# Mamba413/bess

Measured on AMD Instinct MI355X. Metric: candidate subsets solved/sec (n=50k,p=10k,k<=200 LM), higher is better.
Workload: dtype f64; 1 GPU; configs[1]: LM sequential path, Gaussian X n=50000 p=10000, s.list=1..200, GIC, warm start, max_iter=20, is_normal; score_pass=covariance updates (cached Gram columns), collective=none, ranks_with_work=1

## Files before the change

### bess_amd/capi.py

```python
import ctypes
import os
import sys

import numpy as np

_HERE = os.path.dirname(os.path.abspath(__file__))
LIB_PATH = os.environ.get("BESSX_LIB_PATH") or os.path.join(_HERE, "libbessx.so")

_D = ctypes.POINTER(ctypes.c_double)
_I = ctypes.POINTER(ctypes.c_int)
_i = ctypes.c_int
_d = ctypes.c_double
_ll = ctypes.c_longlong
_vp = ctypes.c_void_p

SYMBOLS = [
    "bessx_last_error", "bessx_device_info", "bessx_pywrap_bess", "bessx_bessCpp", "bessx_session_create",
    "bessx_session_destroy", "bessx_session_set_cv", "bessx_session_get_cv_folds", "bessx_session_sequential_path", "bessx_session_gs_path",
    "bessx_session_pgs_path", "bessx_session_get_screening", "bessx_session_get_screening_groups", "bessx_session_get_screening_scores", "bessx_session_score_mode", "bessx_session_counter",
    "bessx_session_trace_enable", "bessx_session_trace_size", "bessx_session_trace_copy_int",
    "bessx_session_trace_copy_double", "bessx_session_get_normalization", "bessx_session_score_pass_stats",
    "bessx_session_enable_kernel_timing", "bessx_session_submodel_steps", "bessx_session_fit", "bessx_session_fit_width", "bessx_session_reset_caches",
    "bessx_session_sequential_path_chain", "bessx_session_cv_eval", "bessx_session_debug_block_stream",
    "bessx_session_set_fill_hook", "bessx_session_set_kpath_chains",
# ... 557 lines not shown
        self._gsize_max = 1
        if gi is not None and gi.size:
            self._gsize_max = int(np.max(np.diff(np.append(gi, self.p))))
        pb = Problem(self.n, self.p, _dp(x), int(x_col_major), _dp(y), _dp(w), data_type, int(is_normal), model_type,
                     algorithm_type, max_iter, int(is_warm_start), _ip(al), al.size, device, _ip(gi),
                     0 if gi is None else gi.size, int(is_screening), int(screening_size), int(score_mode),
                     int(max_sparsity))
        h = _vp()
        if din is not None:
            _check_device_route(lib().bessx_session_create_device(ctypes.byref(h), ctypes.byref(pb), ctypes.byref(din)))
        else:
            _check(lib().bessx_session_create(ctypes.byref(h), ctypes.byref(pb)))
        self._h = h
        self.K = 0
        self.is_warm_start = bool(is_warm_start)
        self.p_kept = lib().bessx_session_get_screening(h, None, 0)

    def score_mode(self):
        return int(lib().bessx_session_score_mode(self._h))

    def counters(self):
        names = {0: "chained_fits", 1: "cg_fallbacks", 2: "passes_over_X", 3: "chained_queued", 7: "cv_side_by_side_rounds",
                 8: "cv_union_fills", 9: "tie_rescues", 10: "cache_restarts", 11: "cv_contexts_dropped",
                 12: "cv_fold_contexts", 13: "shared_wide_fills", 14: "kpath_chunked_paths", 15: "kpath_stitch_refits",
                 16: "kpath_chunk_fills", 17: "kpath_chains_last_path",
                 18: "kpath_stitch_giveups", 19: "group_XTX_ns",
                 22: "kpath_coarse_us",
                 23: "kpath_chunks_us", 24: "kpath_stitch_us", 25: "panel_launches_one_group",
                 26: "panel_ns_one_group", 27: "panel_launches_two_groups", 28: "panel_ns_two_groups",
                 29: "shared_pass_launches", 30: "shared_pass_chain_slots", 31: "shared_pass_partial_batches",
                 32: "own_queue_streams_created_by_the_process", 33: "multi_responses_batched",
                 34: "multi_responses_host", 35: "multi_union_fills", 36: "x_bytes_uploaded_from_host",
                 37: "x_bytes_ingested_on_device", 38: "live_device_bytes_of_the_process",
                 39: "live_pinned_bytes_of_the_process", 40: "allocation_requests_of_the_process"}
        return {n: int(lib().bessx_session_counter(self._h, i)) for i, n in names.items()}

    def screening(self):
        a = np.zeros(self.p_kept, dtype=np.int32)
        lib().bessx_session_get_screening(self._h, _ip(a), a.size)
        return a

    def screening_groups(self):
        n = lib().bessx_session_get_screening_groups(self._h, None, 0)
        a = np.zeros(max(n, 1), dtype=np.int32)
        lib().bessx_session_get_screening_groups(self._h, _ip(a), n)
        return a[:n]

    def screening_scores(self):
        n = lib().bessx_session_get_screening_scores(self._h, None, 0)
        a = np.zeros(max(n, 1))
        lib().bessx_session_get_screening_scores(self._h, _dp(a), n)
        return a[:n]

    def close(self):
        if getattr(self, "_h", None):
            lib().bessx_session_destroy(self._h)
            self._h = None

    def __del__(self):
        try:
            self.close()
        except Exception:
            pass

    def __enter__(self):
        return self

# ... 1872 lines not shown
```

### bess_amd/csrc/bessx_dev.h

```cpp
#ifndef BESSX_DEV_H
#define BESSX_DEV_H

#include <hip/hip_runtime.h>

namespace bessx {

struct FitCtrl {
  int done;
  int l;
  int T0;
  int k_cur;
  int irls_done;
  int irls_steps;
  int info;
  int same_prev;
  double coef0;
  double ll0;
  int d_fresh;
  int irls_last;
  int fast_same;
  int ls_m;
  double ll1;
  int gram_full;
  int cov_nfill;
  int cov_stall;
  int cov_groups;
  int cov_miss;
  int cov_nmiss;
  int serial;
  int sse_valid;
  double sse_dot;
  double sse_nrm;
  unsigned long long snap_seq;
};
static_assert(sizeof(FitCtrl) <= 128, "the published control block is 128 bytes");

// ... 457 lines not shown
hipError_t launch_cov_reduce_compact_sets(const double *part, int p, const int *fcols, const int *slot_of, int *meta,
                                          const CovRowSets &rs, int g0, int ngroups, int nslab, int CS,
                                          const FitCtrl *ctrl, int parked, hipStream_t st);
constexpr int CGB_MAX_K = 4096;
struct CgbState {
  double rr[2];
  double qq;
  int done_step;
  int steps;
};
struct CgbWork {
  double *x, *q, *r[2], *p[2], *ap[2], *part_pq[2], *part_qq;
  CgbState *st;
};
size_t cgb_work_doubles(int kcap);
hipError_t launch_cg_big(const double *G, int p, const int *slot_of, const int *meta, const int *A_new, int k,
                         double ridge, const double *xty, const double *beta_dense, double *work, int kcap, double *sol,
                         FitCtrl *ctrl, int slot, int nsteps, double tol, double yy, hipStream_t st);
struct CovUnion {
  int nf;
  const int *list[8];
  int len[8];
  int on_restart[8];
  int dn;
  const int *const *dlist;
  const int *dlen;
};
hipError_t launch_cov_fill_union(const CovUnion &u, int restart, const int *extras, const double *bd2, int spec_max,
                                 int spec_min, int *slot_of, int *meta, int p, int *fcols, FitCtrl *fill_ctrl,
                                 hipStream_t st, int C = 0);
int cov_streamed_tiles_per_wave();
hipError_t launch_cov_panel(const double *X, const double *aux, long ld, int p, const double *mask, const int *fcols,
                            int g0, int ngroups, int rows_per_slab, int nslab, double *part, const FitCtrl *ctrl,
                            int parked, hipStream_t st);
hipError_t cov_panel_prepare();
hipError_t launch_cov_reduce(const double *part, int p, const int *fcols, const int *slot_of, double *G, int g0,
                             int ngroups, int nslab, const FitCtrl *ctrl, int parked, hipStream_t st,
                             int ex_lo = 0, int ex_hi = 0);
hipError_t launch_rows_permute(const double *X, long ld, int p, const int *perm, long ldp, double *Xp, hipStream_t st);
hipError_t launch_cov_compact(const double *G, int p, const int *slot_of, const int *fcols, int g0, int ngroups,
                              double *GS, int CS, const FitCtrl *ctrl, int parked, hipStream_t st,
                              const double *xtx = nullptr, int *meta = nullptr);
hipError_t launch_cov_d(const double *G, int p, const int *slot_of, const double *xty, const int *A_cur,
                        const double *b_cur, double *d_out, const double *beta_dense, const double *xtx, double n_t,
                        double lambda, const unsigned char *always, double *bd, const unsigned char *inA, double *bmm,
                        const FitCtrl *ctrl, int slot, hipStream_t st);
hipError_t launch_cov_gram(const double *G, int p, const int *slot_of, const int *A_new, int T0, int mt, double *Gt,
                           int *meta, const FitCtrl *ctrl, int slot, hipStream_t st);
hipError_t launch_publish(const unsigned char *dev, unsigned char *host, int ctrl_bytes, size_t off_sse, int n_sse,
                          size_t off_b, size_t off_a, int kcopy, unsigned long long *seq_host, unsigned long long seq,
                          hipStream_t st, const int *count_ptr = nullptr);
hipError_t launch_vec_mul(const double *a, const double *b, long n, double *out, hipStream_t st);
hipError_t launch_part_sum(const double *part, int nrb, int p, double *out, hipStream_t st);
hipError_t launch_fill(double *a, long n, double v, hipStream_t st);
hipError_t launch_gram_cols(const int *A_new, int T0, int mp, int intercept, int rhs_col, int *cols, FitCtrl *ctrl,
                            int slot, const int *A_cur, int allow_skip, hipStream_t st);
hipError_t launch_copy(const double *src, double *dst, long n, hipStream_t st);

}
#endif
```

### bess_amd/csrc/bessx_fit.cpp

```cpp
#include "bessx_host.h"

namespace bessx {

static int score_pass(bessx_session *s, int kind, int rs, int slot, std::vector<std::pair<size_t, bool>> &k1_pairs) {
  if (rs == 0 && shared_pass_applies(s)) {
    if (s->timing) k1_pairs.push_back({(size_t)-1, false});
    if (kind == 2 && s->cox.one_pass)
      return shared_pass_submit(s, nullptr, nullptr, s->part_rs[rs], nullptr, &s->cox, s->ctrl, slot);
    if (kind != 2)
      return shared_pass_submit(s, s->r_rs[rs], kind == 1 ? s->h_rs[rs] : nullptr, s->part_rs[rs],
                                kind == 1 ? s->part2_rs[rs] : nullptr, nullptr, s->ctrl, slot);
  }
  hipEvent_t ea = nullptr, eb = nullptr;
  if (int rc = k1_begin(s, &ea, &eb)) return rc;
  hipError_t e;
  if (kind == 2)
    e = launch_cox_score_pass(s->X, s->ld, s->p, s->U, s->nrb, s->cox, s->part_rs[rs], s->part2_rs[rs], s->ctrl, slot, s->st);
  else
    e = launch_xtv(s->X, s->ld, s->p, s->U, s->r_rs[rs], kind == 1 ? s->h_rs[rs] : nullptr, s->part_rs[rs],
                   kind == 1 ? s->part2_rs[rs] : nullptr, s->ctrl, slot, s->st);
  if (s->timing && e == hipSuccess) {
    e = hipEventRecord(eb, s->st);
    k1_pairs.push_back({s->ev_used - 2, false});
  }
// ... 39 lines not shown
  } else if (e == hipSuccess) {
    int rps_i, nslab_i;
    const int ntask_i = s->gtask_inc_cnt[mt];
    gram_geometry(s, ntask_i * 3, &rps_i, &nslab_i);
    bessx_session::GramCache &gc = s->gcache[rs];
    e = launch_gram_lm_cached(s->X, s->aux, s->ld, s->gcols, s->mask[rs], s->A_new, T0, mt,
                              tasks_full, ntask, rps, nslab, s->gtasks + s->gtask_inc_off[mt],
                              ntask_i, rps_i, nslab_i, s->gpart, s->Gt, s->Rt, s->gsrc, gc.g0, gc.g1, gc.A, gc.meta,
                              s->ctrl, slot, s->st);
    const CholFuse fbz = chol_fallback_only(s);
    if (e == hipSuccess)
      e = launch_chol(s->Gt, T0, mt, lambda, 0, s->xty[rs], s->A_new, s->sol, &s->ctrl->info, s->ctrl, slot, 0, s->st,
                      &fbz);
    if (e == hipSuccess)
      e = launch_sym_fallback(s->Gt, T0, mt, lambda, 0, s->xty[rs], s->A_new, s->sol, &s->ctrl->info, s->ctrl, slot, s->st,
                              &fbz);
  }
  if (e == hipSuccess)
    e = launch_commit(s->ctrl, slot, T0, s->A_new, s->sol, 0, 0, s->A_cur, s->b_cur, s->beta_dense, s->hist,
                      s->hist_beta, s->hist_coef0, s->hist_stride, s->st, s->inA);
  if (e == hipSuccess)
    e = launch_resid_lm(s->X, s->ld, s->n, s->y, s->mask[rs], s->ctrl, slot, s->A_cur, s->b_cur, s->r_rs[rs],
                        s->sse, s->st);
  if (e != hipSuccess) return fail(BESSX_ERR_HIP, std::string("enqueue_lm_slot: ") + hipGetErrorString(e));
  return 0;
}


int enqueue_cov_fill(bessx_session *s, int rs, int ngroups, int parked, const FitCtrl *gate,
                            int gfirst, bool compact, const int *slot_map) {
  bessx_session::CovCache &cv = s->cov[rs];
  const FitCtrl *gc = gate ? gate : s->ctrl;
  const int *smap = slot_map ? slot_map : cv.slot_of;
  for (int g0 = gfirst; g0 < gfirst + ngroups; g0 += COV_SLOT_GROUPS) {
    const int ng = std::min(COV_SLOT_GROUPS, gfirst + ngroups - g0);
    hipEvent_t ea = nullptr, eb = nullptr;
    if (int rc = k1_begin(s, &ea, &eb)) return rc;
    hipError_t e = hipSuccess;
    if (s->cv_shared) {
      const int nsl_all = s->K * s->cvp_nsl;
      e = launch_cov_panel(s->Xp, s->zp, s->ldp, s->p, nullptr, s->cov_fcols, g0, ng, s->cvp_rps, nsl_all, s->cvp_part,
                           gc, parked, s->st);
      if (s->timing && e == hipSuccess) {
        e = hipEventRecord(eb, s->st);
        s->cov_timed.push_back({s->ev_used - 2, g0});
      }
      if (s->K + 1 <= 9 && e == hipSuccess) {
        CovRowSets rsets = {};
        rsets.nr = s->K + 1;
        for (int r = 0; r <= s->K; r++) {
          rsets.G[r] = s->cov[r].G;
          rsets.GS[r] = s->cov[r].GS;
          rsets.xtx[r] = s->xtx[r];
          rsets.ex_lo[r] = r == 0 ? 0 : (r - 1) * s->cvp_nsl;
          rsets.ex_hi[r] = r == 0 ? 0 : r * s->cvp_nsl;
        }
        e = launch_cov_reduce_compact_sets(s->cvp_part, s->p, s->cov_fcols, s->cov[0].slot_of, s->cov[0].meta, rsets, g0, ng,
                                           nsl_all, s->cov_cs, gc, parked, s->st);
      }
      for (int r = 0; r <= s->K && e == hipSuccess && s->K + 1 > 9; r++) {
        bessx_session::CovCache &cr = s->cov[r];
        const int lo = r == 0 ? 0 : (r - 1) * s->cvp_nsl, hi = r == 0 ? 0 : r * s->cvp_nsl;
        e = launch_cov_reduce(s->cvp_part, s->p, s->cov_fcols, cr.slot_of, cr.G, g0, ng, nsl_all, gc, parked, s->st,
                              lo, hi);
        if (e == hipSuccess)
          e = launch_cov_compact(cr.G, s->p, cr.slot_of, s->cov_fcols, g0, ng, cr.GS, s->cov_cs, gc, parked, s->st,
                                 s->xtx[r], cr.meta);
      }
      if (e != hipSuccess) return fail(BESSX_ERR_HIP, std::string("cov panel (shared): ") + hipGetErrorString(e));
      continue;
    }
    e = launch_cov_panel(s->X, s->aux, s->ld, s->p, s->mask[rs], s->cov_fcols, g0, ng, s->cov_rps,
                         s->cov_nslab, s->cov_part, gc, parked, s->st);
    if (s->timing && e == hipSuccess) {
      e = hipEventRecord(eb, s->st);
      s->cov_timed.push_back({s->ev_used - 2, g0});
    }
    if (e == hipSuccess)
      e = launch_cov_reduce(s->cov_part, s->p, s->cov_fcols, smap, cv.G, g0, ng, s->cov_nslab, gc, parked,
                            s->st);
    if (e == hipSuccess && compact)
      e = launch_cov_compact(cv.G, s->p, smap, s->cov_fcols, g0, ng, cv.GS, s->cov_cs, gc, parked, s->st, s->xtx[rs],
                             cv.meta);
    if (e != hipSuccess) return fail(BESSX_ERR_HIP, std::string("cov panel: ") + hipGetErrorString(e));
  }
  return 0;
}

int cov_C_dev(const bessx_session *s) { return s->cov_C - (s->cov_spec - COV_R); }

struct SlotFuse {
  const PubArgs *pub = nullptr;
  bool pub_fused = false;
  bool pub_snapshot = false;
  const PubArgs *attach = nullptr;
  bool attached = false;
  int cont_serial = 0, cont_parent = 0;
  bool cont = false, cont_fused = false;
};

CholFuse cov_fuse_args(bessx_session *s, int rs, int T0, bool force_chol, SlotFuse *sf) {
  bessx_session::CovCache &cv = s->cov[rs];
  CholFuse fz = {cv.G,          cv.slot_of, s->p,         T0,           s->ctrl,        s->A_cur, s->b_cur,
                 s->beta_dense, s->hist,    s->hist_beta, s->hist_coef0, s->hist_stride, s->inA,   s->yy_h[rs],
                 s->part_rs[rs], cv.GS, s->cov_cs,
                 cv.zero, PubArgs{}, s->fb_work, cv.meta + 4};
// ... 1331 lines not shown
```

### bess_amd/csrc/bessx_host.h

```cpp
#ifndef BESSX_HOST_H
#define BESSX_HOST_H
#include <hip/hip_runtime.h>

#include <algorithm>
#include <atomic>
#include <chrono>
#include <cfloat>
#include <cmath>
#include <cstdio>
#include <condition_variable>
#include <cstring>
#include <functional>
#include <mutex>
#include <numeric>
#include <random>
#include <string>
#include <thread>
#include <vector>

#include "../../include/bessx.h"
#include "bessx_dev.h"
#include "bessx_sync.h"

namespace bessx {
// ... 385 lines not shown
    double lambda = 0.0;
    unsigned long long seq = 0;
  } ahead;
  bool chain = true;
  long long chain_queued = 0, chain_hits = 0, chain_dead = 0, chain_mismatch = 0;
  int fit_serial = 0;
  unsigned char *stage_h = nullptr;
  std::vector<double> x_mean_h, x_norm_h;
  std::vector<int> cv_fold;
  std::vector<int> screen_groups, scr_gidx;
  std::vector<double> screen_scores;
  double y_mean_h = 0.0;
  double nullloss = 0.0;
  SparseVec beta;
  double coef0 = 0.0;
  SparseVec beta_init;
  double coef0_init = 0.0;
  int sparsity_level = 0;
  double lambda_level = 0.0;
  int cur_rows = 0;
  int l = 0;
  double sse_train = 0.0, sse_test = 0.0;
  std::vector<SparseVec> cv_init;
  std::vector<int> n_test;
  Trace trace;
  int metric_depth = 0;
  bool timing = false;
  std::vector<hipEvent_t> ev_pool;
  size_t ev_used = 0;
  double k1_seconds = 0.0, k1_bytes = 0.0;
  long long k1_launches = 0;
  double panel_w_seconds[2] = {0.0, 0.0};
  long long panel_w_launches[2] = {0, 0};
  long long n_fits = 0, n_iters = 0;
};

namespace bessx {

static constexpr int COV_R = 32;
static constexpr int COV_SLOT_GROUPS = 2;
static constexpr int COV_CS = 512;

inline Owner &rowset_owner(bessx_session *s, int rs) { return rs == 0 ? s->own : s->cv_own; }

inline int caller_col(const bessx_session *s, int j) { return s->screen_map.empty() ? j : s->screen_map[j]; }

struct SlotFuse;
struct Candidate {
  int T0 = 0;
  double lambda = 0.0;
  SparseVec beta;
  double coef0 = 0.0, loss = 0.0, ic = 0.0;
  int iters = 0;
};
struct PgsArgs;

void ctx_free(bessx_session *c);
void drop_fold_contexts(bessx_session *s);
void session_free(bessx_session *s);
size_t part_elems(const bessx_session *s);
int k1_begin(bessx_session *s, hipEvent_t *a, hipEvent_t *b);
int k1_collect(bessx_session *s, const std::vector<std::pair<size_t, bool>> &pairs);
int cov_collect(bessx_session *s, int nfill);
int alloc_gram_cache(bessx_session *s);
int alloc_cov_cache(bessx_session *s, bool share_map = false);
int reset_path_caches(bessx_session *s);
// ... 57 lines not shown
  std::vector<int> i, A;
  std::vector<double> d, b;
};
bool mc_engine_applies(const bessx_session *s);
int mc_sse_by_residual(bessx_session *c, hipStream_t st, const int *idx, const double *val, int T0, double coef0, double *out);
int mc_contexts(bessx_session *s, int n);
void kchains_contexts(const bessx_session *s, std::vector<bessx_session *> *out);
bessx_session *mc_context(bessx_session *s, int i);
int mc_engine(bessx_session *s, const int *seq, int ns, std::vector<McJob> &jobs, int nrec, double lambda, int width,
              McRecords &rec, std::vector<int> &takeover, long long *fills);
void kchains_quiesce(bessx_session *s);
int kchunks_prepare(bessx_session *s, int ns, bool link, bool link_warm = false);
hipError_t cox_alloc(bessx_session *s);
int chain_ctx_create(bessx_session *ps, bessx_session **out, bool own_queue = true);
int prefill_begin(bessx_session *s, const int *cols, int ncols, int append);
int glm_geometry(bessx_session *s, int T0, int *mt, int *mp, int *ntask, int *ntiles, int *rps, int *nslab);
int enqueue_glm_head(bessx_session *s, int slot, int T0, double lambda, int rs, bool skip_k1,
                            std::vector<std::pair<size_t, bool>> &k1_pairs);
int enqueue_glm_irls_step(bessx_session *s, int slot, int t, int T0, double lambda, int rs);
int enqueue_glm_tail(bessx_session *s, int slot, int T0, int rs);
int cox_reserve(bessx_session *s, int T0);
int enqueue_cox_head(bessx_session *s, int slot, int T0, double lambda, int rs, bool skip_k1,
                            std::vector<std::pair<size_t, bool>> &k1_pairs);
int enqueue_cox_newton(bessx_session *s, int slot, int t, int T0, double lambda, int rs);
int enqueue_cox_tail(bessx_session *s, int slot, int T0, int rs);
PubArgs publish_args(bessx_session *s, int kcopy, int buf, unsigned long long *seq);
PubArgs publish_from_snapshot(const PubArgs &tail);
int publish_flush(bessx_session *s);
int publish_launch(bessx_session *s, const PubArgs &pa);
int publish_enqueue(bessx_session *s, int kcopy, int buf, unsigned long long *seq);
int publish_wait(bessx_session *s, int buf, unsigned long long want);
bool ctx_stream_create(int device, hipStream_t *st, int leave_out = 0, int stride = 1);
long long ctx_streams_created();
void ctx_stream_destroy(hipStream_t st);
bool ctx_streams_own_queue(int device);
int stream_wait_bounded(bessx_session *s, hipStream_t st, const char *what);
int read_results(bessx_session *s, int kcopy = -1);
int algorithm_fit_grouped(bessx_session *s);
int enqueue_chained(bessx_session *s, const bessx_session::Hint &hint, int rs, int parent, int buf, int batch,
                           double parent_lambda, int parent_T0);
int algorithm_fit(bessx_session *s);
void fold_contexts_invalidate(bessx_session *s);
bool side_by_side_applies(const bessx_session *s, int T0);
int fold_fits_side_by_side(bessx_session *s, double *out, const std::vector<int> *only = nullptr,
                                  double *per_fold = nullptr);
double metric_train_loss_value(const bessx_session *s);
double metric_fold_test_loss(const bessx_session *s, int k);
int metric_train_loss(bessx_session *s, double *out);
int metric_test_loss(bessx_session *s, double *out);
int metric_ic(bessx_session *s, int ic_type, int is_cv, double *out);
void denormalize(const bessx_session *s, SparseVec &b, double &coef0, bool gs_variant);
int run_fit(bessx_session *s, int T0, double lambda, const SparseVec &beta_init, double coef0_init);
void store_candidate(bessx_session *s, bessx_path_result *res, const Candidate &c, bool gs_variant);
void store_best(bessx_session *s, bessx_path_result *res, const Candidate &c, bool gs_variant);
bool chain_row_matches(const bessx_session *s, const bessx_path_chain *ch, int row, const Candidate &c);
int sequential_path(bessx_session *s, const int *seq, int ns, const double *lam, int nl, int ic_type,
                           int is_cv, bessx_path_result *res, bessx_path_chain *chain = nullptr);
int gs_path(bessx_session *s, int s_min, int s_max, int ic_type, int is_cv, bessx_path_result *res);
int pgs_path(bessx_session *s, int s_min, int s_max, double lmin, double lmax, int powell_path, int nlambda,
                    int ic_type, int is_cv, bessx_path_result *res);
int settle_device_chain(bessx_session *s);
int run_path(bessx_session *s, bool gs, const int *seq, int ns, const double *lam, int nl, int s_min,
                    int s_max, int ic_type, int is_cv, bessx_path_result *res, const PgsArgs *pgs = nullptr,
                    bessx_path_chain *chain = nullptr);
int need_device();
int upload_padded(Owner &sc, const double *x, int n, int p, int ld_in, int U, double **dX, long *ld_out);
// ... 7 lines not shown
```

### bess_amd/csrc/bessx_k_cov.hip

```cpp
#include "bessx_kdev.hpp"

namespace bessx {

constexpr int COV_NJ = 4;

#ifdef BESSX_PANEL_CLOCK
#define PCLK_BEGIN()                                                  \
  const unsigned long long pclk_t0_ = __builtin_amdgcn_s_memtime();   \
  const unsigned long long pclk_r0_ = __builtin_amdgcn_s_memrealtime()
#define PCLK_END(tag)                                                                                           \
  do {                                                                                                          \
    asm volatile("s_waitcnt vmcnt(0) lgkmcnt(0)" ::: "memory");                                                 \
    if (blockIdx.x == 7 && threadIdx.x == 0) {                                                                  \
      const unsigned long long dt_ = __builtin_amdgcn_s_memtime() - pclk_t0_;                                   \
      const unsigned long long dr_ = __builtin_amdgcn_s_memrealtime() - pclk_r0_;                               \
      printf("PCLK %s cycles %llu ticks100MHz %llu MHz %.0f\n", tag, dt_, dr_, dr_ ? 100.0 * (double)dt_ / (double)dr_ : 0.0); \
    }                                                                                                           \
  } while (0)
#else
#define PCLK_BEGIN()
#define PCLK_END(tag)
#endif

__device__ __forceinline__ bool cov_gate(const FitCtrl *ctrl, int slot) {
  if (ctrl->done) return false;
  if (slot == 0) return ctrl->l == 0;
  return ctrl->l == slot - 1 && !ctrl->same_prev;
}


__global__ void __launch_bounds__(256) k_cov_need(const int *__restrict__ list, int len,
                                                  const double *__restrict__ bd, double *__restrict__ bd2, int p,
                                                  int *__restrict__ slot_of, int *__restrict__ meta, int C,
// ... 139 lines not shown
  for (int i = tot + tid; i < padded; i += 256) fcols[i] = -1;
  for (int i = nm + tid; i < tot; i += 256) slot_of[fcols[i]] = count + i;
  if (tid == 0) {
    meta[0] = count + tot;
    if (restart) {
      meta[3] += 1;
      meta[4] = 0;
    }
    fill_ctrl->cov_stall = 1;
    fill_ctrl->cov_nfill = padded;
    fill_ctrl->cov_groups += padded / COV_R;
    fill_ctrl->k_cur = count + tot;
    fill_ctrl->cov_nmiss = restart;
  }
}

#ifndef DP_PAD
#define DP_PAD 2
#endif
constexpr int DP_RB = 32;
constexpr int DP_LD = DP_RB + DP_PAD;
constexpr int DP_SC = 128;
template <bool MASKED, int NT>
__device__ __forceinline__ void cov_dp_body(const double *__restrict__ X, const double *__restrict__ aux, long ld,
                                            int p, const double *__restrict__ mask, const int *__restrict__ fcols,
                                            int g0, int rows_per_slab, int nslab, int njg,
                                            double *__restrict__ part, double *smem) {
  constexpr int NS = DP_SC / 32;
  constexpr int NL = NS + NT / 2;
  constexpr int COLS = DP_SC + 16 * NT;
  constexpr size_t BUF = (size_t)COLS * DP_LD;
  constexpr int NA = NT / 2, NB = 2;
  const int njg2 = (njg + 1) / 2;
  const int slab = blockIdx.x / njg2, jb = blockIdx.x - slab * njg2;
  const int tid = threadIdx.x, lane = tid & 63, wv = __builtin_amdgcn_readfirstlane(tid >> 6), c = lane & 15, q = lane >> 4;
  const int ta = NT == 4 ? 2 * (wv & 3) : wv, tb = NT == 4 ? 2 * (wv >> 2) : 0;
  const int ru = tid & 15, cbase = tid >> 4;
  const int jc = min(jb * DP_SC + cbase, p - 1);
  const double *sx = X + (size_t)jc * ld + 2 * ru;
  const long sstride = 32 * ld;
  const int ilim = jb * DP_SC + cbase < p ? (p - 1 - (jb * DP_SC + cbase)) / 32 : 0;
  const double *src[NT / 2];
#pragma unroll
  for (int i = 0; i < NT / 2; i++) src[i] = gram_col(X, aux, ld, fcols[g0 * COV_R + i * 32 + cbase]) + 2 * ru;
  const long r_begin = (long)slab * rows_per_slab, r_end = min(r_begin + rows_per_slab, ld);
  const int nchunk = (int)((r_end - r_begin + DP_RB - 1) / DP_RB);
  d2 stA[NL], stB[NL], mA = d2{1.0, 1.0}, mB = d2{1.0, 1.0};
#define DP_LOAD1(st, ms, r, i)                                                                                  \
  do {                                                                                                          \
    if ((i) < NS)                                                                                               \
      st[i] = __builtin_nontemporal_load(reinterpret_cast<const d2 *>(sx + min((i), ilim) * sstride + (r)));    \
    else                                                                                                        \
      st[i] = *reinterpret_cast<const d2 *>(src[(i) >= NS ? (i)-NS : 0] + (r));                                 \
    if (MASKED && (i) == NL - 1) ms = *reinterpret_cast<const d2 *>(mask + (r) + 2 * ru);                       \
  } while (0)
#define DP_STORE1(buf, st, ms, i)                                                                               \
  do {                                                                                                          \
    d2 v__ = st[i];                                                                                             \
    if (MASKED && (i) >= NS) v__ = v__ * ms;                                                                    \
    *reinterpret_cast<d2 *>((buf) + 2 * ru + (size_t)((i)*32 + cbase) * DP_LD) = v__;                           \
  } while (0)
  d4 acc[NA * NB];
#pragma unroll
  for (int t = 0; t < NA * NB; t++) acc[t] = d4{0.0, 0.0, 0.0, 0.0};
  const size_t offa = (size_t)(ta * 16 + c) * DP_LD + 4 * q, offb = (size_t)(DP_SC + tb * 16 + c) * DP_LD + 4 * q;
  struct Ops {
    d2 a0[NA], a1[NA], b0[NB], b1[NB];
  };
  auto read_ops = [&](const double *rows, Ops &o) {
#pragma unroll
    for (int a = 0; a < NA; a++) {
      o.a0[a] = *reinterpret_cast<const d2 *>(rows + offa + (size_t)a * 16 * DP_LD);
      o.a1[a] = *reinterpret_cast<const d2 *>(rows + offa + (size_t)a * 16 * DP_LD + 2);
    }
#pragma unroll
    for (int t = 0; t < NB; t++) {
      o.b0[t] = *reinterpret_cast<const d2 *>(rows + offb + (size_t)t * 16 * DP_LD);
      o.b1[t] = *reinterpret_cast<const d2 *>(rows + offb + (size_t)t * 16 * DP_LD + 2);
    }
  };
#define DP_MFMA(o, j)                                                                                           \
  do {                                                                                                          \
    _Pragma("unroll") for (int a__ = 0; a__ < NA; a__++) {                                                    \
      const double av__ = (j) == 0 ? (o).a0[a__].x : ((j) == 1 ? (o).a0[a__].y : ((j) == 2 ? (o).a1[a__].x : (o).a1[a__].y)); \
      _Pragma("unroll") for (int t__ = 0; t__ < NB; t__++) {                                                  \
        const double bv__ = (j) == 0 ? (o).b0[t__].x : ((j) == 1 ? (o).b0[t__].y : ((j) == 2 ? (o).b1[t__].x : (o).b1[t__].y)); \
        acc[a__ * NB + t__] = __builtin_amdgcn_mfma_f64_16x16x4f64(av__, bv__, acc[a__ * NB + t__], 0, 0, 0);   \
      }                                                                                                         \
    }                                                                                                           \
  } while (0)
  static_assert(DP_RB == 32, "two row steps per chunk");
#define DP_STEP(o, s, nxt, st, ms, rload)                                                                       \
  do {                                                                                                          \
    int n__ = (s) * NL;                                                                                         \
    _Pragma("unroll") for (int j__ = 0; j__ < 4; j__++) {                                                     \
      DP_MFMA(o, j__);                                                                                          \
                                         \
      const int due__ = (2 * NL * ((s) * 4 + j__ + 1)) / (4 * (DP_RB / 16));                                    \
      _Pragma("unroll") for (int k__ = 0; k__ < 2 * NL; k__++) {                                              \
        if (k__ >= n__ && k__ < due__) {                                                                        \
          if (k__ < NL)                                                                                         \
            DP_STORE1(nxt, st, ms, k__);                                                                        \
          else                                                                                                  \
            DP_LOAD1(st, ms, rload, k__ - NL);                                                                  \
        }                                                                                                       \
      }                                                                                                         \
      n__ = due__;                                                                                              \
      __builtin_amdgcn_sched_barrier(0);                                                                        \
    }                                                                                                           \
  } while (0)
#define DP_CHUNK(cur, nxt, st, ms, rload)                                                                       \
  do {                                                                                                          \
    read_ops((cur) + 16, ob);                                                                                   \
    __builtin_amdgcn_sched_barrier(0);                                                                          \
    DP_STEP(oa, 0, nxt, st, ms, rload);                                                                         \
    __syncthreads();                                                                                            \
    read_ops(nxt, oa);                                                                                          \
    __builtin_amdgcn_sched_barrier(0);                                                                          \
    DP_STEP(ob, 1, nxt, st, ms, rload);                                                                         \
  } while (0)
  double *buf0 = smem, *buf1 = smem + BUF;
  const long r_last = r_begin + (long)(nchunk - 1) * DP_RB;
#pragma unroll
  for (int i = 0; i < NL; i++) DP_LOAD1(stA, mA, r_begin, i);
#pragma unroll
  for (int i = 0; i < NL; i++) DP_STORE1(buf0, stA, mA, i);
  {
    const long r1 = min(r_begin + DP_RB, r_last), r2 = min(r_begin + 2 * DP_RB, r_last);
#pragma unroll
    for (int i = 0; i < NL; i++) DP_LOAD1(stB, mB, r1, i);
#pragma unroll
    for (int i = 0; i < NL; i++) DP_LOAD1(stA, mA, r2, i);
  }
  __syncthreads();
  Ops oa, ob;
  read_ops(buf0, oa);
  for (int k = 0; k < nchunk; k += 2) {
    {
      const long rl = min(r_begin + (long)(k + 3) * DP_RB, r_last);
      DP_CHUNK(buf0, buf1, stB, mB, rl);
    }
    if (k + 1 >= nchunk) break;
    {
      const long rl = min(r_begin + (long)(k + 4) * DP_RB, r_last);
      DP_CHUNK(buf1, buf0, stA, mA, rl);
    }
  }
#undef DP_STEP
#undef DP_CHUNK
#undef DP_MFMA
#undef DP_LOAD1
#undef DP_STORE1
  const size_t tiles_per_slab = (size_t)njg * COV_NJ * 2;
#pragma unroll
  for (int a = 0; a < NA; a++) {
    const int jg = 2 * jb + ((ta + a) >> 2);
    if (jg < njg) {
#pragma unroll
      for (int t = 0; t < NB; t++) {
        double *out = part + (((size_t)((tb + t) >> 1) * nslab + slab) * tiles_per_slab + (size_t)(jg * COV_NJ + ((ta + a) & 3)) * 2 + ((tb + t) & 1)) * 256;
        *reinterpret_cast<d4 *>(out + lane * 4) = acc[a * NB + t];
      }
    }
  }
}

template <bool MASKED>
__global__ void __launch_bounds__(512, 1) k_cov_panel_dp(const double *__restrict__ X, const double *__restrict__ aux,
                                                         long ld, int p, const double *__restrict__ mask,
                                                         const int *__restrict__ fcols, int g0, int ngroups,
                                                         int rows_per_slab, int nslab, int njg,
                                                         double *__restrict__ part, const FitCtrl *__restrict__ ctrl,
                                                         int big) {
  KT(5);
  if (big ? !ctrl->cov_stall : (ctrl->done || ctrl->l != 0)) return;
  const int nfill = ctrl->cov_nfill;
  if (g0 * COV_R >= nfill) return;
  extern __shared__ double smem[];
  PCLK_BEGIN();
  if (ngroups >= 2 && (g0 + 1) * COV_R < nfill)
    cov_dp_body<MASKED, 4>(X, aux, ld, p, mask, fcols, g0, rows_per_slab, nslab, njg, part, smem);
  else
    cov_dp_body<MASKED, 2>(X, aux, ld, p, mask, fcols, g0, rows_per_slab, nslab, njg, part, smem);
  PCLK_END("dp");
}

__device__ __forceinline__ void cov_reduce_body(const double *__restrict__ part, int g0, int ngroups, int nslab,
                                                int njg, int p, const int *__restrict__ fcols,
                                                const int *__restrict__ slot_of, double *__restrict__ G,
                                                const FitCtrl *__restrict__ ctrl, int big,
                                                int ex_lo, int ex_hi) {
  if (big ? !ctrl->cov_stall : (ctrl->done || ctrl->l != 0)) return;
  const int gl = blockIdx.y;
  if (gl >= ngroups || (g0 + gl) * COV_R >= ctrl->cov_nfill) return;
  const size_t tiles_per_slab = (size_t)njg * COV_NJ * 2;
  const int tile = blockIdx.x, e = threadIdx.x;
  double s = 0.0;
// ... 216 lines not shown
hipError_t launch_cov_publish_slots(const int *fcols, const int *slot_w, int *slot_of, const FitCtrl *ctrl, hipStream_t st) {
  hipLaunchKernelGGL(k_cov_publish_slots, dim3(1), dim3(256), 0, st, fcols, slot_w, slot_of, ctrl);
  LAUNCH_CHECK();
  return hipSuccess;
}

hipError_t launch_cov_fill_list(int *fcols, const int *extras, const double *bd2, int *slot_of, int *meta,
                                FitCtrl *ctrl, int parked, hipStream_t st, int spec_max, int spec, int spec_min) {
  if (spec_min <= 0) spec_min = spec_max / 2;
  hipLaunchKernelGGL(k_cov_fill_list, dim3(1), dim3(256), 0, st, fcols, extras, bd2, slot_of, meta, ctrl, parked,
                     spec_max, spec, spec_min);
  LAUNCH_CHECK();
  return hipSuccess;
}

hipError_t launch_cov_resume(FitCtrl *ctrl, hipStream_t st) {
  hipLaunchKernelGGL(k_cov_resume, dim3(1), dim3(1), 0, st, ctrl);
  LAUNCH_CHECK();
  return hipSuccess;
}

hipError_t launch_cov_fill_union(const CovUnion &u, int restart, const int *extras, const double *bd2, int spec_max,
                                 int spec_min, int *slot_of, int *meta, int p, int *fcols, FitCtrl *fill_ctrl,
                                 hipStream_t st, int C) {
  if (u.nf < 1 || u.nf > 8 || u.dn < 0 || (u.dn > 0 && (!u.dlist || !u.dlen)) || spec_max > 64 || spec_min < 0 || spec_min > spec_max) return hipErrorInvalidValue;
  hipLaunchKernelGGL(k_cov_fill_union, dim3(1), dim3(256), 0, st, u, restart, extras, bd2, spec_max, spec_min, slot_of, meta, p,
                     fcols, fill_ctrl, C);
  LAUNCH_CHECK();
  return hipSuccess;
}

int cov_streamed_tiles_per_wave() { return COV_NJ; }

hipError_t launch_cov_panel(const double *X, const double *aux, long ld, int p, const double *mask, const int *fcols,
                            int g0, int ngroups, int rows_per_slab, int nslab, double *part, const FitCtrl *ctrl,
                            int parked, hipStream_t st) {
  if (ngroups < 1 || ngroups > 2) return hipErrorInvalidValue;
  const int pt = (p + 15) / 16, njg = (pt + COV_NJ - 1) / COV_NJ;
  const size_t ldsd = (size_t)2 * (DP_SC + 64) * DP_LD * sizeof(double);
  const long nbd = (long)nslab * ((njg + 1) / 2);
  if (mask)
    hipLaunchKernelGGL(k_cov_panel_dp<true>, dim3((unsigned)nbd), dim3(512), ldsd, st, X, aux, ld, p, mask, fcols, g0,
                       ngroups, rows_per_slab, nslab, njg, part, ctrl, parked);
  else
    hipLaunchKernelGGL(k_cov_panel_dp<false>, dim3((unsigned)nbd), dim3(512), ldsd, st, X, aux, ld, p, mask, fcols, g0,
                       ngroups, rows_per_slab, nslab, njg, part, ctrl, parked);
  LAUNCH_CHECK();
  return hipSuccess;
}

hipError_t cov_panel_prepare() {
  const int ldsd = (int)((size_t)2 * (DP_SC + 64) * DP_LD * sizeof(double));
  hipError_t e = hipFuncSetAttribute(reinterpret_cast<const void *>(&k_cov_panel_dp<true>),
                                     hipFuncAttributeMaxDynamicSharedMemorySize, ldsd);
  if (e != hipSuccess) return e;
  return hipFuncSetAttribute(reinterpret_cast<const void *>(&k_cov_panel_dp<false>),
                             hipFuncAttributeMaxDynamicSharedMemorySize, ldsd);
}

hipError_t launch_cov_reduce(const double *part, int p, const int *fcols, const int *slot_of, double *G, int g0,
                             int ngroups, int nslab, const FitCtrl *ctrl, int parked, hipStream_t st, int ex_lo,
                             int ex_hi) {
  const int pt = (p + 15) / 16, njg = (pt + COV_NJ - 1) / COV_NJ;
  hipLaunchKernelGGL(k_cov_reduce, dim3(njg * COV_NJ * 2, ngroups), dim3(256), 0, st, part, g0, ngroups, nslab, njg, p,
                     fcols, slot_of, G, ctrl, 0, parked, ex_lo, ex_hi);
  LAUNCH_CHECK();
  return hipSuccess;
}

hipError_t launch_cov_reduce_compact_sets(const double *part, int p, const int *fcols, const int *slot_of, int *meta,
                                          const CovRowSets &rs, int g0, int ngroups, int nslab, int CS,
                                          const FitCtrl *ctrl, int parked, hipStream_t st) {
  if (rs.nr < 1 || rs.nr > 9) return hipErrorInvalidValue;
  const int pt = (p + 15) / 16, njg = (pt + COV_NJ - 1) / COV_NJ;
  hipLaunchKernelGGL(k_cov_reduce_sets, dim3(njg * COV_NJ * 2, ngroups, rs.nr), dim3(256), 0, st, part, g0, ngroups,
                     nslab, njg, p, fcols, slot_of, rs, ctrl, parked);
  LAUNCH_CHECK();
  hipLaunchKernelGGL(k_cov_compact_sets, dim3((p + 255) / 256, ngroups, rs.nr), dim3(256), 0, st, rs, p, slot_of, fcols,
// ... 59 lines not shown
```

### bess_amd/csrc/bessx_session.cpp

```cpp
#include "bessx_host.h"

namespace bessx {

thread_local std::string g_err;
thread_local int g_marginal_fit_variant = 0;



void ctx_free(bessx_session *c) {
  if (!c) return;
  if (c->st) (void)hipStreamSynchronize(c->st);
  c->own.release();
  if (c->st) ctx_stream_destroy(c->st);
  delete c;
}

void drop_fold_contexts(bessx_session *s) {
  if (s->fold_pool) {
    s->fold_pool->stop();
    if (!s->fold_pool->broken) delete s->fold_pool;
    s->fold_pool = nullptr;
  }
  for (bessx_session *c : s->fold_ctx) ctx_free(c);
  s->fold_ctx.clear();
// ... 157 lines not shown
    for (auto &o : g_own_streams)
      if (!o.in_use && o.device == device && o.leave_out == leave_out && o.stride == stride) {
        o.in_use = true;
        *st = o.st;
        return true;
      }
    if (g_own_streams.size() >= std::max(cap, OWN_QUEUE_CAP)) {
      for (size_t i = 0; i < g_own_streams.size(); i++)
        if (!g_own_streams[i].in_use) {
          (void)hipStreamDestroy(g_own_streams[i].st);
          g_own_streams.erase(g_own_streams.begin() + (long)i);
          break;
        }
      if (g_own_streams.size() >= std::max(cap, OWN_QUEUE_CAP)) return false;
    }
  }
  hipDeviceProp_t prop;
  if (hipGetDeviceProperties(&prop, device) != hipSuccess || prop.multiProcessorCount <= 0) return false;
  std::vector<uint32_t> mask((size_t)(prop.multiProcessorCount + 31) / 32, 0xffffffffu);
  if (prop.multiProcessorCount % 32) mask.back() = (1u << (prop.multiProcessorCount % 32)) - 1u;
  for (int i = 0; i < leave_out; i++) {
    const int bit = (int)(((long)i * std::max(1, stride)) % prop.multiProcessorCount);
    mask[(size_t)bit / 32] &= ~(1u << (bit % 32));
  }
  if (hipExtStreamCreateWithCUMask(st, (uint32_t)mask.size(), mask.data()) != hipSuccess) {
    (void)hipGetLastError();
    *st = nullptr;
    return false;
  }
  std::lock_guard<std::mutex> lk(g_own_mu);
  g_own_streams.push_back({*st, device, leave_out, stride, true});
  g_own_created++;
  return true;
}

bool ctx_streams_own_queue(int device) {
  static std::mutex mu;
  static std::vector<int> known;
  std::lock_guard<std::mutex> lk(mu);
  if (device < 0) return false;
  if ((int)known.size() <= device) known.resize((size_t)device + 1, -1);
  if (known[(size_t)device] < 0) {
    hipStream_t st = nullptr;
    const bool ok = ctx_stream_create(device, &st);
    if (ok) ctx_stream_destroy(st);
    known[(size_t)device] = ok ? 1 : 0;
  }
  return known[(size_t)device] == 1;
}

int stream_wait_bounded(bessx_session *s, hipStream_t st, const char *what) {
  const auto t0 = std::chrono::steady_clock::now();
  for (unsigned spins = 0;; spins++) {
    const hipError_t q = hipStreamQuery(st);
    if (q == hipSuccess) return 0;
    if (q != hipErrorNotReady) return fail(BESSX_ERR_HIP, std::string(what) + ": " + hipGetErrorString(q));
    if (std::chrono::duration<double>(std::chrono::steady_clock::now() - t0).count() > s->wait_deadline_s)
      return fail(BESSX_ERR_HIP, std::string(what) + ": the stream did not drain within " +
                                     std::to_string(s->wait_deadline_s) + " s (BESSX_WAIT_TIMEOUT_S) -- the session can "
                                     "only be destroyed now");
    if (spins > 2000) std::this_thread::sleep_for(std::chrono::microseconds(50));
  }
}

int reset_path_caches(bessx_session *s) {
  kchains_quiesce(s);
// ... 814 lines not shown
      if (C >= 2 * COV_R + s->cov_spec) {
        s->cov_mode = true;
        s->cov_C = (int)C;
        const int pt = (p + 15) / 16, njg = (pt + cov_streamed_tiles_per_wave() - 1) / cov_streamed_tiles_per_wave();
        long ns = 1, rps = ld;
        long panel_blocks = 0;
        {
          const long conc = 256;
          double best = 1e300;
          const long ns_max = std::max<long>(1, std::min<long>(64, ld / 256));
          for (long t = 1; t <= ns_max; t++) {
            const long r = ((ld + t - 1) / t + 63) / 64 * 64, used = (ld + r - 1) / r;
            const long blocks = (long)((njg + 1) / 2) * used;
            const double cost = (double)((blocks + conc - 1) / conc) * (double)r * (blocks < conc ? 2.0 : 1.0);
            if (cost < best) {
              best = cost;
              ns = used;
              rps = r;
              panel_blocks = blocks;
            }
          }
        }
        s->cov_panel_blocks = (int)std::min<long>(panel_blocks, 1 << 30);
        s->cov_rps = (int)rps;
        s->cov_nslab = (int)ns;
        HIPT(s->own.alloc(&s->cov_part, (size_t)COV_SLOT_GROUPS * ns * njg * cov_streamed_tiles_per_wave() * 2 * 256));
        HIPT(s->own.alloc(&s->bd2, (size_t)p));
        HIPT(s->own.zeros(&s->inA, (size_t)p));
        HIPT(s->own.alloc(&s->cov_bmm, (size_t)3 * ((p + 31) / 32)));
        HIPT(s->own.alloc(&s->cov_fcols, (size_t)s->capA + 4 * COV_R));
        HIPT(s->own.alloc(&s->cov_extras, (size_t)2 * COV_R));
        TRY(alloc_cov_cache(s));
        HIPT(cov_panel_prepare());
        if (const char *ev = test_hook("cov_solver")) s->cov_cg = std::string(ev) != "chol";
        if (const char *ev = test_hook("fuse")) s->fuse = std::string(ev) != "0";
        if (const char *ev = test_hook("fuse_sel")) s->fuse_sel = std::string(ev) != "0";
        if (const char *ev = test_hook("defer_publish")) s->defer_pub = std::string(ev) != "0";
        if (!s->fuse) s->defer_pub = false;
        if (const char *ev = test_hook("cg_layout")) s->cg_by_rows = std::string(ev) != "tiles";
        if (const char *ev = test_hook("cov_cs")) s->cov_cs = std::min(COV_CS, std::max(1, std::atoi(ev)));
      } else if (mode == 2) {
        return bail(fail(BESSX_ERR_ARG, "covariance score mode: p too large for the Gram column cache"));
      }
    }
  }
  HIPT(s->own.alloc(&s->idcols, (size_t)capA + 16));
  if (s->model_type == 4) HIPT(cox_alloc(s));
  if (s->model_type == 1) {
    TRY(prepare_rowset(s, 0));
    if (const char *ev = test_hook("path_group_xtx")) s->path_group_xtx = std::string(ev) != "0";
  }
  HIPT(hipStreamSynchronize(s->st));
#undef TRY
#undef HIPT
  *out = s;
  return BESSX_OK;
}

static int fetch_device_vector(const char *what, const void *data, int dtype, long long stride, int n, int device,
                               hipStream_t caller, std::vector<double> &host) {
  int dev = -1;
  if (int rc = check_device_matrix(what, data, dtype, stride, 0, n, 1, &dev)) return rc;
  if (dev != device) return fail(BESSX_ERR_ARG, std::string(what) + ": memory of another device than the session's");
  const long long ld = ((long long)n + 127) / 128 * 128;
  Owner sc;
  double *d = nullptr;
// ... 524 lines not shown
    case 4: return 0;
    case 5:
    case 6: return 0;
    case 7: return s->cv_rounds;
    case 8: return s->cv_union_fills;
    case 9: return s->cov_tie_rescues;
    case 11: return s->cv_ctx_dropped;
    case 12: return (long long)s->fold_ctx.size();
    case 13: return s->shared_wide_fills;
    case 14: return s->kch_paths;
    case 15: return s->kch_refits;
    case 16: return s->kch_chunk_fills;
    case 17: return s->kch_last_chains;
    case 18: return s->kch_giveups;
    case 19: {
      if (s->xtx_ev_pending && s->xtx_ev[0] && s->xtx_ev[1]) {
        float ms = 0.f;
        bessx_session *w = const_cast<bessx_session *>(s);
        if (hipEventSynchronize(s->xtx_ev[1]) == hipSuccess && hipEventElapsedTime(&ms, s->xtx_ev[0], s->xtx_ev[1]) == hipSuccess)
          w->group_xtx_ns = (long long)(1e6 * (double)ms);
        w->xtx_ev_pending = false;
      }
      return s->group_xtx_ns;
    }
    case 20:
    case 21: return 0;
    case 22: return (long long)(1e6 * s->kch_t[0]);
    case 23: return (long long)(1e6 * s->kch_t[1]);
    case 24: return (long long)(1e6 * s->kch_t[2]);
    case 25: return s->panel_w_launches[0];
    case 26: return (long long)(1e9 * s->panel_w_seconds[0]);
    case 27: return s->panel_w_launches[1];
    case 28: return (long long)(1e9 * s->panel_w_seconds[1]);
    case 29: return s->sp_launches;
    case 30: return s->sp_chain_slots;
    case 31: return s->sp_partial;
    case 32: return ctx_streams_created();
    case 33: return s->multi_batched;
    case 34: return s->multi_host;
    case 35: return s->multi_fills;
    case 36: return s->x_host_bytes;
    case 37: return s->x_dev_bytes;
    case 38: return Ledger::device_bytes.load();
    case 39: return Ledger::pinned_bytes.load();
    case 40: return Ledger::requests.load();
    case 10: {
      if (s->cov.empty()) return 0;
      int m[8] = {0, 0, 0, 0, 0, 0, 0, 0};
      if (hipSetDevice(s->device) != hipSuccess || hipStreamSynchronize(s->st) != hipSuccess ||
          hipMemcpy(m, s->cov[0].meta, sizeof(m), hipMemcpyDeviceToHost) != hipSuccess)
        return -1;
      return m[3];
    }
    default: return -1;
  }
}

int bessx_session_get_screening(const bessx_session *s, int *columns, int cap) {
  if (!s) return 0;
  for (int j = 0; j < s->p && j < cap && columns; j++) columns[j] = caller_col(s, j);
  return s->p;
}

int bessx_session_get_screening_groups(const bessx_session *s, int *groups, int cap) {
  if (!s) return 0;
  const int cnt = (int)s->screen_groups.size();
// ... 31 lines not shown
```

Baseline: 19140 candidates/s.

## Make covariance panel kernel persistent with grid-stride work items

The covariance panel kernel now launches at most one workgroup per compute unit and walks (slab, column-block) items in a grid-stride loop. It carries the double-buffered prefetch across item boundaries, so the next item's loads overlap the current item's tail, and it stores each item's accumulators when that item finishes. This targets launch tail effects and pipeline refill cost from many short workgroups. The cost is more complex control flow, possible extra register pressure, and load imbalance when items do not divide evenly across workgroups.

```diff
diff --git a/bess_amd/capi.py b/bess_amd/capi.py
--- a/bess_amd/capi.py
+++ b/bess_amd/capi.py
@@ -613,7 +613,8 @@
                  32: "own_queue_streams_created_by_the_process", 33: "multi_responses_batched",
                  34: "multi_responses_host", 35: "multi_union_fills", 36: "x_bytes_uploaded_from_host",
                  37: "x_bytes_ingested_on_device", 38: "live_device_bytes_of_the_process",
-                 39: "live_pinned_bytes_of_the_process", 40: "allocation_requests_of_the_process"}
+                 39: "live_pinned_bytes_of_the_process", 40: "allocation_requests_of_the_process",
+                 41: "panel_workgroups_last_launch", 42: "panel_items_last_launch"}
         return {n: int(lib().bessx_session_counter(self._h, i)) for i, n in names.items()}
 
     def screening(self):
diff --git a/bess_amd/csrc/bessx_dev.h b/bess_amd/csrc/bessx_dev.h
--- a/bess_amd/csrc/bessx_dev.h
+++ b/bess_amd/csrc/bessx_dev.h
@@ -2,6 +2,8 @@
 #define BESSX_DEV_H
 
 #include <hip/hip_runtime.h>
+
+#include "bessx_panel_items.h"
 
 namespace bessx {
 
@@ -525,7 +527,8 @@
 int cov_streamed_tiles_per_wave();
 hipError_t launch_cov_panel(const double *X, const double *aux, long ld, int p, const double *mask, const int *fcols,
                             int g0, int ngroups, int rows_per_slab, int nslab, double *part, const FitCtrl *ctrl,
-                            int parked, hipStream_t st);
+                            int parked, hipStream_t st, int grid);
+int cov_panel_items(int p, int nslab);
 hipError_t cov_panel_prepare();
 hipError_t launch_cov_reduce(const double *part, int p, const int *fcols, const int *slot_of, double *G, int g0,
                              int ngroups, int nslab, const FitCtrl *ctrl, int parked, hipStream_t st,
diff --git a/bess_amd/csrc/bessx_fit.cpp b/bess_amd/csrc/bessx_fit.cpp
--- a/bess_amd/csrc/bessx_fit.cpp
+++ b/bess_amd/csrc/bessx_fit.cpp
@@ -95,6 +95,12 @@
   bessx_session::CovCache &cv = s->cov[rs];
   const FitCtrl *gc = gate ? gate : s->ctrl;
   const int *smap = slot_map ? slot_map : cv.slot_of;
+  const int units = ctx_stream_units(s->device, s->st);
+  auto grid_of = [&](int nslab) {
+    s->panel_last_items = cov_panel_items(s->p, nslab);
+    s->panel_last_grid = panel_grid(s->panel_last_items, units, s->panel_grid_cap);
+    return s->panel_last_grid;
+  };
   for (int g0 = gfirst; g0 < gfirst + ngroups; g0 += COV_SLOT_GROUPS) {
     const int ng = std::min(COV_SLOT_GROUPS, gfirst + ngroups - g0);
     hipEvent_t ea = nullptr, eb = nullptr;
@@ -103,7 +109,7 @@
     if (s->cv_shared) {
       const int nsl_all = s->K * s->cvp_nsl;
       e = launch_cov_panel(s->Xp, s->zp, s->ldp, s->p, nullptr, s->cov_fcols, g0, ng, s->cvp_rps, nsl_all, s->cvp_part,
-                           gc, parked, s->st);
+                           gc, parked, s->st, grid_of(nsl_all));
       if (s->timing && e == hipSuccess) {
         e = hipEventRecord(eb, s->st);
         s->cov_timed.push_back({s->ev_used - 2, g0});
@@ -134,7 +140,7 @@
       continue;
     }
     e = launch_cov_panel(s->X, s->aux, s->ld, s->p, s->mask[rs], s->cov_fcols, g0, ng, s->cov_rps,
-                         s->cov_nslab, s->cov_part, gc, parked, s->st);
+                         s->cov_nslab, s->cov_part, gc, parked, s->st, grid_of(s->cov_nslab));
     if (s->timing && e == hipSuccess) {
       e = hipEventRecord(eb, s->st);
       s->cov_timed.push_back({s->ev_used - 2, g0});
diff --git a/bess_amd/csrc/bessx_host.h b/bess_amd/csrc/bessx_host.h
--- a/bess_amd/csrc/bessx_host.h
+++ b/bess_amd/csrc/bessx_host.h
@@ -441,6 +441,8 @@
   long long k1_launches = 0;
   double panel_w_seconds[2] = {0.0, 0.0};
   long long panel_w_launches[2] = {0, 0};
+  int panel_last_grid = 0, panel_last_items = 0;
+  int panel_grid_cap = 0;
   long long n_fits = 0, n_iters = 0;
 };
 
@@ -564,6 +566,7 @@
 int publish_wait(bessx_session *s, int buf, unsigned long long want);
 bool ctx_stream_create(int device, hipStream_t *st, int leave_out = 0, int stride = 1);
 long long ctx_streams_created();
+int ctx_stream_units(int device, hipStream_t st);
 void ctx_stream_destroy(hipStream_t st);
 bool ctx_streams_own_queue(int device);
 int stream_wait_bounded(bessx_session *s, hipStream_t st, const char *what);
diff --git a/bess_amd/csrc/bessx_k_cov.hip b/bess_amd/csrc/bessx_k_cov.hip
--- a/bess_amd/csrc/bessx_k_cov.hip
+++ b/bess_amd/csrc/bessx_k_cov.hip
@@ -1,4 +1,5 @@
 #include "bessx_kdev.hpp"
+#include "bessx_panel_items.h"
 
 namespace bessx {
 
@@ -204,24 +205,52 @@
   constexpr size_t BUF = (size_t)COLS * DP_LD;
   constexpr int NA = NT / 2, NB = 2;
   const int njg2 = (njg + 1) / 2;
-  const int slab = blockIdx.x / njg2, jb = blockIdx.x - slab * njg2;
+  const int G = (int)gridDim.x, items = panel_item_count(nslab, njg2);
   const int tid = threadIdx.x, lane = tid & 63, wv = __builtin_amdgcn_readfirstlane(tid >> 6), c = lane & 15, q = lane >> 4;
   const int ta = NT == 4 ? 2 * (wv & 3) : wv, tb = NT == 4 ? 2 * (wv >> 2) : 0;
   const int ru = tid & 15, cbase = tid >> 4;
-  const int jc = min(jb * DP_SC + cbase, p - 1);
-  const double *sx = X + (size_t)jc * ld + 2 * ru;
   const long sstride = 32 * ld;
-  const int ilim = jb * DP_SC + cbase < p ? (p - 1 - (jb * DP_SC + cbase)) / 32 : 0;
+  auto chunks_of = [&](int slab) {
+    const long rb = (long)slab * rows_per_slab;
+    return (int)((min(rb + rows_per_slab, ld) - rb + DP_RB - 1) / DP_RB);
+  };
+  const double *cp[NS];
+  auto columns_of = [&](int jb) {
+    const int j0 = jb * DP_SC + cbase;
+    const double *sx = X + (size_t)min(j0, p - 1) * ld + 2 * ru;
+    const int ilim = j0 < p ? (p - 1 - j0) / 32 : 0;
+#pragma unroll
+    for (int i = 0; i < NS; i++) cp[i] = sx + min(i, ilim) * sstride;
+  };
+  int item_l = panel_item_of((int)blockIdx.x, 0, G), item_c = item_l;
+  if (item_c >= items) return;
+  PanelItem it_c = panel_item_split(item_c, njg2);
+  int rem_c = chunks_of(it_c.slab), rem_l = rem_c;
+  long r_l = (long)it_c.slab * rows_per_slab;
+  columns_of(it_c.jb);
+  auto advance_load = [&]() {
+    r_l += DP_RB;
+    if (--rem_l == 0) {
+      if (item_l + G < items) {
+        item_l += G;
+        const PanelItem it = panel_item_split(item_l, njg2);
+        r_l = (long)it.slab * rows_per_slab;
+        rem_l = chunks_of(it.slab);
+        columns_of(it.jb);
+      } else {
+        r_l -= DP_RB;
+        rem_l = 1;
+      }
+    }
+  };
   const double *src[NT / 2];
 #pragma unroll
   for (int i = 0; i < NT / 2; i++) src[i] = gram_col(X, aux, ld, fcols[g0 * COV_R + i * 32 + cbase]) + 2 * ru;
-  const long r_begin = (long)slab * rows_per_slab, r_end = min(r_begin + rows_per_slab, ld);
-  const int nchunk = (int)((r_end - r_begin + DP_RB - 1) / DP_RB);
   d2 stA[NL], stB[NL], mA = d2{1.0, 1.0}, mB = d2{1.0, 1.0};
 #define DP_LOAD1(st, ms, r, i)                                                                                  \
   do {                                                                                                          \
     if ((i) < NS)                                                                                               \
-      st[i] = __builtin_nontemporal_load(reinterpret_cast<const d2 *>(sx + min((i), ilim) * sstride + (r)));    \
+      st[i] = __builtin_nontemporal_load(reinterpret_cast<const d2 *>(cp[(i) < NS ? (i) : 0] + (r)));           \
     else                                                                                                        \
       st[i] = *reinterpret_cast<const d2 *>(src[(i) >= NS ? (i)-NS : 0] + (r));                                 \
     if (MASKED && (i) == NL - 1) ms = *reinterpret_cast<const d2 *>(mask + (r) + 2 * ru);                       \
@@ -281,6 +310,7 @@
       __builtin_amdgcn_sched_barrier(0);                                                                        \
     }                                                                                                           \
   } while (0)
+#define DP_FENCE() asm volatile("" ::: "memory")
 #define DP_CHUNK(cur, nxt, st, ms, rload)                                                                       \
   do {                                                                                                          \
     read_ops((cur) + 16, ob);                                                                                   \
@@ -290,51 +320,64 @@
     read_ops(nxt, oa);                                                                                          \
     __builtin_amdgcn_sched_barrier(0);                                                                          \
     DP_STEP(ob, 1, nxt, st, ms, rload);                                                                         \
+    DP_FENCE();                                                                                                 \
   } while (0)
   double *buf0 = smem, *buf1 = smem + BUF;
-  const long r_last = r_begin + (long)(nchunk - 1) * DP_RB;
-#pragma unroll
-  for (int i = 0; i < NL; i++) DP_LOAD1(stA, mA, r_begin, i);
+  const size_t tiles_per_slab = (size_t)njg * COV_NJ * 2;
+  auto store_item = [&](const PanelItem &it) {
+#pragma unroll
+    for (int a = 0; a < NA; a++) {
+      const int jg = 2 * it.jb + ((ta + a) >> 2);
+      if (jg < njg) {
+#pragma unroll
+        for (int t = 0; t < NB; t++) {
+          double *out = part + (((size_t)((tb + t) >> 1) * nslab + it.slab) * tiles_per_slab + (size_t)(jg * COV_NJ + ((ta + a) & 3)) * 2 + ((tb + t) & 1)) * 256;
+          *reinterpret_cast<d4 *>(out + lane * 4) = acc[a * NB + t];
+        }
+      }
+    }
+  };
+#pragma unroll
+  for (int i = 0; i < NL; i++) DP_LOAD1(stA, mA, r_l, i);
+  advance_load();
 #pragma unroll
   for (int i = 0; i < NL; i++) DP_STORE1(buf0, stA, mA, i);
-  {
-    const long r1 = min(r_begin + DP_RB, r_last), r2 = min(r_begin + 2 * DP_RB, r_last);
-#pragma unroll
-    for (int i = 0; i < NL; i++) DP_LOAD1(stB, mB, r1, i);
-#pragma unroll
-    for (int i = 0; i < NL; i++) DP_LOAD1(stA, mA, r2, i);
-  }
+#pragma unroll
+  for (int i = 0; i < NL; i++) DP_LOAD1(stB, mB, r_l, i);
+  DP_FENCE();
+  advance_load();
+#pragma unroll
+  for (int i = 0; i < NL; i++) DP_LOAD1(stA, mA, r_l, i);
+  DP_FENCE();
+  advance_load();
   __syncthreads();
   Ops oa, ob;
   read_ops(buf0, oa);
-  for (int k = 0; k < nchunk; k += 2) {
-    {
-      const long rl = min(r_begin + (long)(k + 3) * DP_RB, r_last);
-      DP_CHUNK(buf0, buf1, stB, mB, rl);
-    }
-    if (k + 1 >= nchunk) break;
-    {
-      const long rl = min(r_begin + (long)(k + 4) * DP_RB, r_last);
-      DP_CHUNK(buf1, buf0, stA, mA, rl);
-    }
-  }
+#define DP_ITEM_END()                                                                                           \
+  if (--rem_c == 0) {                                                                                           \
+    store_item(it_c);                                                                                           \
+    item_c += G;                                                                                                \
+    more = item_c < items;                                                                                      \
+    _Pragma("unroll") for (int t__ = 0; t__ < NA * NB; t__++) acc[t__] = d4{0.0, 0.0, 0.0, 0.0};              \
+    it_c = panel_item_split(more ? item_c : 0, njg2);                                                           \
+    rem_c = more ? chunks_of(it_c.slab) : 0x7fffffff;                                                           \
+  }
+  bool more = true;
+  do {
+    DP_CHUNK(buf0, buf1, stB, mB, r_l);
+    advance_load();
+    DP_ITEM_END();
+    DP_CHUNK(buf1, buf0, stA, mA, r_l);
+    advance_load();
+    DP_ITEM_END();
+  } while (more);
+#undef DP_ITEM_END
 #undef DP_STEP
 #undef DP_CHUNK
+#undef DP_FENCE
 #undef DP_MFMA
 #undef DP_LOAD1
 #undef DP_STORE1
-  const size_t tiles_per_slab = (size_t)njg * COV_NJ * 2;
-#pragma unroll
-  for (int a = 0; a < NA; a++) {
-    const int jg = 2 * jb + ((ta + a) >> 2);
-    if (jg < njg) {
-#pragma unroll
-      for (int t = 0; t < NB; t++) {
-        double *out = part + (((size_t)((tb + t) >> 1) * nslab + slab) * tiles_per_slab + (size_t)(jg * COV_NJ + ((ta + a) & 3)) * 2 + ((tb + t) & 1)) * 256;
-        *reinterpret_cast<d4 *>(out + lane * 4) = acc[a * NB + t];
-      }
-    }
-  }
 }
 
 template <bool MASKED>
@@ -617,18 +660,24 @@
 
 int cov_streamed_tiles_per_wave() { return COV_NJ; }
 
+int cov_panel_items(int p, int nslab) {
+  const int pt = (p + 15) / 16, njg = (pt + COV_NJ - 1) / COV_NJ;
+  return panel_item_count(nslab, (njg + 1) / 2);
+}
+
 hipError_t launch_cov_panel(const double *X, const double *aux, long ld, int p, const double *mask, const int *fcols,
                             int g0, int ngroups, int rows_per_slab, int nslab, double *part, const FitCtrl *ctrl,
-                            int parked, hipStream_t st) {
+                            int parked, hipStream_t st, int grid) {
   if (ngroups < 1 || ngroups > 2) return hipErrorInvalidValue;
   const int pt = (p + 15) / 16, njg = (pt + COV_NJ - 1) / COV_NJ;
+  const int items = cov_panel_items(p, nslab);
+  if (grid < 1 || grid > items || rows_per_slab < 1 || (long)(nslab - 1) * rows_per_slab >= ld) return hipErrorInvalidValue;
   const size_t ldsd = (size_t)2 * (DP_SC + 64) * DP_LD * sizeof(double);
-  const long nbd = (long)nslab * ((njg + 1) / 2);
   if (mask)
-    hipLaunchKernelGGL(k_cov_panel_dp<true>, dim3((unsigned)nbd), dim3(512), ldsd, st, X, aux, ld, p, mask, fcols, g0,
+    hipLaunchKernelGGL(k_cov_panel_dp<true>, dim3((unsigned)grid), dim3(512), ldsd, st, X, aux, ld, p, mask, fcols, g0,
                        ngroups, rows_per_slab, nslab, njg, part, ctrl, parked);
   else
-    hipLaunchKernelGGL(k_cov_panel_dp<false>, dim3((unsigned)nbd), dim3(512), ldsd, st, X, aux, ld, p, mask, fcols, g0,
+    hipLaunchKernelGGL(k_cov_panel_dp<false>, dim3((unsigned)grid), dim3(512), ldsd, st, X, aux, ld, p, mask, fcols, g0,
                        ngroups, rows_per_slab, nslab, njg, part, ctrl, parked);
   LAUNCH_CHECK();
   return hipSuccess;
diff --git a/bess_amd/csrc/bessx_panel_items.h b/bess_amd/csrc/bessx_panel_items.h
--- /dev/null
+++ b/bess_amd/csrc/bessx_panel_items.h
@@ -0,0 +1,35 @@
+#pragma once
+
+#if defined(__HIPCC__) || defined(__CUDACC__)
+#define BESSX_HD __host__ __device__
+#else
+#define BESSX_HD
+#endif
+
+namespace bessx {
+
+struct PanelItem {
+  int slab, jb;
+};
+
+BESSX_HD inline int panel_item_count(int nslab, int blocks_per_slab) { return nslab * blocks_per_slab; }
+
+BESSX_HD inline int panel_grid(int items, int units, int cap) {
+  int g = items;
+  if (units > 0 && g > units) g = units;
+  if (cap > 0 && g > cap) g = cap;
+  return g < 1 ? 1 : g;
+}
+
+BESSX_HD inline int panel_item_of(int w, int t, int G) { return w + t * G; }
+
+BESSX_HD inline int panel_items_of_workgroup(int items, int G, int w) { return w < items ? (items - 1 - w) / G + 1 : 0; }
+
+BESSX_HD inline PanelItem panel_item_split(int item, int blocks_per_slab) {
+  PanelItem it;
+  it.slab = item / blocks_per_slab;
+  it.jb = item - it.slab * blocks_per_slab;
+  return it;
+}
+
+}
diff --git a/bess_amd/csrc/bessx_session.cpp b/bess_amd/csrc/bessx_session.cpp
--- a/bess_amd/csrc/bessx_session.cpp
+++ b/bess_amd/csrc/bessx_session.cpp
@@ -213,6 +213,30 @@
   g_own_streams.push_back({*st, device, leave_out, stride, true});
   g_own_created++;
   return true;
+}
+
+int ctx_stream_units(int device, hipStream_t st) {
+  static std::mutex mu;
+  static std::vector<int> cus;
+  int n = 0;
+  {
+    std::lock_guard<std::mutex> lk(mu);
+    if (device < 0) return 0;
+    if ((int)cus.size() <= device) cus.resize((size_t)device + 1, 0);
+    if (cus[(size_t)device] == 0) {
+      hipDeviceProp_t prop;
+      if (hipGetDeviceProperties(&prop, device) != hipSuccess || prop.multiProcessorCount <= 0) {
+        (void)hipGetLastError();
+        return 0;
+      }
+      cus[(size_t)device] = prop.multiProcessorCount;
+    }
+    n = cus[(size_t)device];
+  }
+  std::lock_guard<std::mutex> lk(g_own_mu);
+  for (auto &o : g_own_streams)
+    if (o.st == st && o.in_use) return std::max(1, n - std::min(o.leave_out, n));
+  return n;
 }
 
 bool ctx_streams_own_queue(int device) {
@@ -1093,6 +1117,7 @@
         HIPT(s->own.alloc(&s->cov_extras, (size_t)2 * COV_R));
         TRY(alloc_cov_cache(s));
         HIPT(cov_panel_prepare());
+        if (const char *ev = test_hook("panel_grid")) s->panel_grid_cap = std::max(0, std::atoi(ev));
         if (const char *ev = test_hook("cov_solver")) s->cov_cg = std::string(ev) != "chol";
         if (const char *ev = test_hook("fuse")) s->fuse = std::string(ev) != "0";
         if (const char *ev = test_hook("fuse_sel")) s->fuse_sel = std::string(ev) != "0";
@@ -1683,6 +1708,8 @@
     case 26: return (long long)(1e9 * s->panel_w_seconds[0]);
     case 27: return s->panel_w_launches[1];
     case 28: return (long long)(1e9 * s->panel_w_seconds[1]);
+    case 41: return s->panel_last_grid;
+    case 42: return s->panel_last_items;
     case 29: return s->sp_launches;
     case 30: return s->sp_chain_slots;
     case 31: return s->sp_partial;
```

After: 19410 candidates/s, median of 6. 1.4% higher.
